# SebastianBitsch/SRGAN-ST

Measured on AMD Instinct MI355X. Metric: HR images/sec (96px x4, B=16/GPU) G+D+ST-loss step, higher is better.
Workload: dtype f32; 1 GPU; srgan_x4_hr96_b16_G+D+ST-loss step: adv+mse+st, D updated every step (train.py:116-164; BASELINE metric); global_batch=16, hr=96, lr=24, parallelism=dp1, hip_graph=True, d_update_interval=1, d_sr_forward=run: all three discriminator forwards of train.py:136,155,158

## Files before the change

srgan-st_amd/csrc/linear.hip:

```cpp
#include "common.h"

typedef float f32x4 __attribute__((ext_vector_type(4)));

namespace {
constexpr int NT = 256;
constexpr int MAXM = 64;

__global__ __launch_bounds__(NT) void linear_fwd_kernel(const float* __restrict__ x, const float* __restrict__ w,
                                                        float* __restrict__ slab, int M, int N, int K, int kslice) {
  __shared__ float red[4][MAXM][17];
  const int wave = __builtin_amdgcn_readfirstlane(threadIdx.x >> 6), lane = threadIdx.x & 63;
  const int lj = lane & 15, lq = lane >> 4;
  const int n0 = blockIdx.x * 16;
  const int kb = blockIdx.y * kslice, ke = min(K, kb + kslice);
  const int mt = (M + 15) / 16;
  f32x4 acc[4];
#pragma unroll
  for (int t = 0; t < 4; ++t) acc[t] = f32x4{0.f, 0.f, 0.f, 0.f};
  const int n = min(n0 + lj, N - 1);
  const float* wrow = w + (size_t)n * K;
  for (int k = kb + wave * 16; k < ke; k += 64) {
    const int kk = k + 4 * lq;
    f32x4 bv = {0.f, 0.f, 0.f, 0.f};
    if (kk + 3 < ke) {
      bv = *reinterpret_cast<const f32x4*>(wrow + kk);
    } else {
#pragma unroll
      for (int j = 0; j < 4; ++j)
        if (kk + j < ke) bv[j] = wrow[kk + j];
    }
#pragma unroll
    for (int t = 0; t < 4; ++t) {
      if (t < mt) {
        const int m = t * 16 + lj;
        f32x4 av = {0.f, 0.f, 0.f, 0.f};
        if (m < M) {
          if (kk + 3 < ke) {
            av = *reinterpret_cast<const f32x4*>(x + (size_t)m * K + kk);
          } else {
#pragma unroll
            for (int j = 0; j < 4; ++j)
              if (kk + j < ke) av[j] = x[(size_t)m * K + kk + j];
          }
        }
#pragma unroll
        for (int j = 0; j < 4; ++j) acc[t] = __builtin_amdgcn_mfma_f32_16x16x4f32(av[j], bv[j], acc[t], 0, 0, 0);
      }
    }
  }
#pragma unroll
  for (int t = 0; t < 4; ++t)
#pragma unroll
    for (int r = 0; r < 4; ++r) red[wave][t * 16 + 4 * lq + r][lj] = acc[t][r];
  __syncthreads();
  for (int i = threadIdx.x; i < M * 16; i += NT) {
    const int m = i >> 4, j = i & 15;
    if (n0 + j < N)
      slab[((size_t)blockIdx.y * M + m) * N + n0 + j] = red[0][m][j] + red[1][m][j] + red[2][m][j] + red[3][m][j];
  }
}

__global__ __launch_bounds__(NT) void linear_reduce_kernel(const float* __restrict__ slab, const float* __restrict__ bias,
                                                           float* __restrict__ y, int nslab, int M, int N) {
  const int total = M * N;
  for (int i = blockIdx.x * NT + threadIdx.x; i < total; i += gridDim.x * NT) {
    float t = bias ? bias[i % N] : 0.f;
    for (int s = 0; s < nslab; ++s) t += slab[(size_t)s * total + i];
    y[i] = t;
  }
}

template <int MT>
__global__ __launch_bounds__(NT) void linear_dgrad_kernel(const float* __restrict__ dy, const float* __restrict__ w,
                                                          float* __restrict__ dx, int M, int N, int K, int C, int HW) {
  __shared__ float red[4][16][65];
  const int wave = __builtin_amdgcn_readfirstlane(threadIdx.x >> 6), lane = threadIdx.x & 63;
  const int lj = lane & 15, lq = lane >> 4;
  const int k0 = blockIdx.x * 64;
  const int nper = ((N + 3) / 4 + 3) / 4 * 4;
  const int nb = wave * nper, ne = min(N, nb + nper);
  f32x4 acc[MT][4];
#pragma unroll
  for (int mt = 0; mt < MT; ++mt)
#pragma unroll
    for (int t = 0; t < 4; ++t) acc[mt][t] = f32x4{0.f, 0.f, 0.f, 0.f};
  int n = nb;
  if (k0 + 64 <= K) {
    constexpr int U = MT == 1 ? 8 : 4;
    const float* wcol = w + k0 + 4 * lj;
    for (; n + 4 * U <= ne; n += 4 * U) {
      f32x4 bv[U];
      float av[MT][U];
#pragma unroll
      for (int u = 0; u < U; ++u) {
        const int nn = n + 4 * u + lq;
        bv[u] = *reinterpret_cast<const f32x4*>(wcol + (size_t)nn * K);
#pragma unroll
        for (int mt = 0; mt < MT; ++mt) {
          const int m = mt * 16 + lj;
          av[mt][u] = m < M ? dy[(size_t)m * N + nn] : 0.f;
        }
      }
#pragma unroll
      for (int u = 0; u < U; ++u)
#pragma unroll
        for (int mt = 0; mt < MT; ++mt)
#pragma unroll
          for (int t = 0; t < 4; ++t) acc[mt][t] = __builtin_amdgcn_mfma_f32_16x16x4f32(av[mt][u], bv[u][t], acc[mt][t], 0, 0, 0);
    }
  }
  for (; n < ne; n += 4) {
    const int nn = n + lq;
    f32x4 bv = {0.f, 0.f, 0.f, 0.f};
    if (nn < ne) {
      const int kk = k0 + 4 * lj;
      if (kk + 3 < K) {
        bv = *reinterpret_cast<const f32x4*>(w + (size_t)nn * K + kk);
      } else {
#pragma unroll
        for (int j = 0; j < 4; ++j)
          if (kk + j < K) bv[j] = w[(size_t)nn * K + kk + j];
      }
    }
#pragma unroll
    for (int mt = 0; mt < MT; ++mt) {
      const int m = mt * 16 + lj;
      const float av = (nn < ne && m < M) ? dy[(size_t)m * N + nn] : 0.f;
#pragma unroll
      for (int t = 0; t < 4; ++t) acc[mt][t] = __builtin_amdgcn_mfma_f32_16x16x4f32(av, bv[t], acc[mt][t], 0, 0, 0);
    }
  }
#pragma unroll
  for (int mt = 0; mt < MT; ++mt) {
    __syncthreads();
#pragma unroll
    for (int t = 0; t < 4; ++t)
#pragma unroll
      for (int r = 0; r < 4; ++r) red[wave][4 * lq + r][4 * lj + t] = acc[mt][t][r];
    __syncthreads();
    for (int i = threadIdx.x; i < 16 * 64; i += NT) {
      const int mm = i >> 6, kc = i & 63, mg = mt * 16 + mm, k = k0 + kc;
      if (mg < M && k < K) {
        const float v = red[0][mm][kc] + red[1][mm][kc] + red[2][mm][kc] + red[3][mm][kc];
        const size_t o = HW > 0 ? (size_t)mg * K + (size_t)(k % HW) * C + k / HW : (size_t)mg * K + k;
        dx[o] = v;
      }
    }
  }
}

__global__ __launch_bounds__(NT) void linear_wgrad_kernel(const float* __restrict__ dy, const float* __restrict__ x,
                                                          float* __restrict__ dw, int M, int N, int K, int accumulate) {
  __shared__ float sdy[MAXM][16];
  const int n0 = blockIdx.y * 16;
  for (int i = threadIdx.x; i < M * 16; i += NT) {
    const int m = i >> 4, j = i & 15;
    sdy[m][j] = (n0 + j < N) ? dy[(size_t)m * N + n0 + j] : 0.f;
  }
  __syncthreads();
  const int k = (blockIdx.x * NT + threadIdx.x) * 4;
  if (k >= K) return;
  const bool vec = (K & 3) == 0;
  f32x4 acc[16];
#pragma unroll
  for (int j = 0; j < 16; ++j) acc[j] = f32x4{0.f, 0.f, 0.f, 0.f};
  for (int m = 0; m < M; ++m) {
    f32x4 xv = {0.f, 0.f, 0.f, 0.f};
    if (vec) {
      xv = *reinterpret_cast<const f32x4*>(x + (size_t)m * K + k);
    } else {
#pragma unroll
      for (int j = 0; j < 4; ++j)
        if (k + j < K) xv[j] = x[(size_t)m * K + k + j];
    }
#pragma unroll
    for (int j = 0; j < 16; ++j) acc[j] += sdy[m][j] * xv;
  }
#pragma unroll
  for (int j = 0; j < 16; ++j) {
    if (n0 + j >= N) break;
    float* d = dw + (size_t)(n0 + j) * K + k;
    if (vec) {
      f32x4 o = acc[j];
      if (accumulate) o += *reinterpret_cast<f32x4*>(d);
      *reinterpret_cast<f32x4*>(d) = o;
    } else {
      for (int q = 0; q < 4; ++q)
        if (k + q < K) d[q] = accumulate ? d[q] + acc[j][q] : acc[j][q];
    }
  }
}

typedef float f32x16 __attribute__((ext_vector_type(16)));
__global__ __launch_bounds__(NT) void linear_wgrad_mfma_kernel(const float* __restrict__ dy, const float* __restrict__ x,
                                                               float* __restrict__ dw, int M, int N, int K, int accumulate) {
  const int wave = threadIdx.x >> 6, lane = threadIdx.x & 63;
  const int li = lane & 31, lh = lane >> 5;
  const int k0 = (blockIdx.x * 4 + wave) * 32, n0 = blockIdx.y * 64;
  if (k0 >= K) return;
  f32x16 acc0, acc1;
#pragma unroll
  for (int r = 0; r < 16; ++r) acc0[r] = acc1[r] = 0.f;
  const float* xp = x + (size_t)lh * K + k0 + li;
  const float* dp = dy + (size_t)lh * N + n0 + li;
  const int steps = (M + 1) >> 1;
  for (int j0 = 0; j0 < steps; j0 += 8) {
    float xv[8], d0[8], d1[8];
#pragma unroll
    for (int u = 0; u < 8; ++u) {
      const int m = 2 * (j0 + u) + lh;
      const bool ok = j0 + u < steps && m < M;
      xv[u] = ok ? xp[(size_t)2 * (j0 + u) * K] : 0.f;
      d0[u] = ok ? dp[(size_t)2 * (j0 + u) * N] : 0.f;
      d1[u] = ok ? dp[(size_t)2 * (j0 + u) * N + 32] : 0.f;
    }
#pragma unroll
    for (int u = 0; u < 8; ++u) {
      acc0 = __builtin_amdgcn_mfma_f32_32x32x2f32(d0[u], xv[u], acc0, 0, 0, 0);
      acc1 = __builtin_amdgcn_mfma_f32_32x32x2f32(d1[u], xv[u], acc1, 0, 0, 0);
    }
  }
#pragma unroll
  for (int r = 0; r < 16; ++r) {
    const int row = (r & 3) + 8 * (r >> 2) + 4 * lh;
    float* d = dw + (size_t)(n0 + row) * K + k0 + li;
    float* e = d + (size_t)32 * K;
    if (accumulate) {
      *d += acc0[r];
      *e += acc1[r];
    } else {
      *d = acc0[r];
      *e = acc1[r];
    }
  }
}

__global__ void colsum_small_kernel(const float* __restrict__ dy, float* __restrict__ db, int M, int N, int accumulate) {
  const int n = blockIdx.x * blockDim.x + threadIdx.x;
  if (n < N) {
    float t = 0.f;
    for (int m = 0; m < M; ++m) t += dy[(size_t)m * N + n];
    db[n] = accumulate ? db[n] + t : t;
  }
}

__global__ __launch_bounds__(NT) void head_fwd_kernel(const float* __restrict__ h, const float* __restrict__ w,
                                                      const float* __restrict__ b, float* __restrict__ y, int M, int N, int K,
                                                      float slope) {
  __shared__ float red[NT / 64];
  const int m = blockIdx.x / N, n = blockIdx.x - m * N;
  float s = 0.f;
  for (int k = threadIdx.x; k < K; k += NT) {
    float v = h[(size_t)m * K + k];
    v = v > 0.f ? v : v * slope;
    s = fmaf(v, w[(size_t)n * K + k], s);
  }
  s = block_sum<NT>(s, red);
  if (threadIdx.x == 0) y[(size_t)m * N + n] = s + (b ? b[n] : 0.f);
}

constexpr int HB_ROWS = 8;
__global__ __launch_bounds__(NT) void head_bwd_kernel(const float* __restrict__ h, const float* __restrict__ w,
                                                      const float* __restrict__ dy, float* __restrict__ dh,
                                                      float* __restrict__ dw, float* __restrict__ db, int M, int N, int K,
                                                      float slope, int accumulate) {
  const int k = blockIdx.x * NT + threadIdx.x;
  const int m0 = blockIdx.y * HB_ROWS, m1 = min(M, m0 + HB_ROWS);
  if (k < K) {
    float hv[HB_ROWS];
#pragma unroll
    for (int i = 0; i < HB_ROWS; ++i) hv[i] = m0 + i < m1 ? h[(size_t)(m0 + i) * K + k] : 0.f;
    float t[HB_ROWS];
#pragma unroll
    for (int i = 0; i < HB_ROWS; ++i) t[i] = 0.f;
    for (int n = 0; n < N; ++n) {
      const float wv = w[(size_t)n * K + k];
#pragma unroll
      for (int i = 0; i < HB_ROWS; ++i)
        if (m0 + i < m1) t[i] = fmaf(dy[(size_t)(m0 + i) * N + n], wv, t[i]);
    }
#pragma unroll
    for (int i = 0; i < HB_ROWS; ++i)
      if (m0 + i < m1) dh[(size_t)(m0 + i) * K + k] = hv[i] > 0.f ? t[i] : t[i] * slope;
    if (dw && blockIdx.y == 0) {
      for (int n = 0; n < N; ++n) {
        float a = 0.f;
        for (int mb = 0; mb < M; mb += HB_ROWS) {
          float v[HB_ROWS];
#pragma unroll
          for (int i = 0; i < HB_ROWS; ++i) v[i] = mb + i < M ? h[(size_t)(mb + i) * K + k] : 0.f;
#pragma unroll
          for (int i = 0; i < HB_ROWS; ++i) {
            if (mb + i >= M) break;
            const float x = v[i] > 0.f ? v[i] : v[i] * slope;
            a = fmaf(dy[(size_t)(mb + i) * N + n], x, a);
          }
        }
        dw[(size_t)n * K + k] = accumulate ? dw[(size_t)n * K + k] + a : a;
      }
    }
  }
  if (db && blockIdx.x == 0 && blockIdx.y == 0 && threadIdx.x < N) {
    float t = 0.f;
    for (int m = 0; m < M; ++m) t += dy[(size_t)m * N + threadIdx.x];
    db[threadIdx.x] = accumulate ? db[threadIdx.x] + t : t;
  }
}

__global__ __launch_bounds__(NT) void flatten_act_kernel(const float* __restrict__ y, const float* __restrict__ scale,
                                                         const float* __restrict__ shift, float slope, int act,
                                                         float* __restrict__ flat, int B, int HW, int C, int gB) {
  const int64_t total = (int64_t)B * HW * C;
  for (int64_t i = blockIdx.x * (int64_t)NT + threadIdx.x; i < total; i += (int64_t)gridDim.x * NT) {
    const int c = (int)(i % C);
    const int64_t p = i / C;
    const int hw = (int)(p % HW);
    const int64_t b = p / HW;
    float v = y[i];
    if (scale) {
      const int gc = (int)(b / gB) * C + c;
      v = fmaf(v, scale[gc], shift[gc]);
    }
    if (act) v = v > 0.f ? v : v * slope;
    flat[(b * C + c) * HW + hw] = v;
  }
}
}

SST_API int sst_linear_ksplit(int M, int N, int K) {
  int ks = 1024 / ((N + 15) / 16);
  if (ks < 1) ks = 1;
  while (ks > 1 && K / ks < 256) ks >>= 1;
  return ks;
}

SST_API int sst_linear_fwd(const float* x, const float* w, const float* bias, float* y, float* slab, int M, int N, int K,
                           void* stream) {
  SST_REQUIRE(x && w && y && slab && M > 0 && M <= MAXM && N > 0 && K > 0, "sst_linear_fwd: bad argument (M=%d)", M);
  const int ks = sst_linear_ksplit(M, N, K);
  const int kslice = ((K + ks - 1) / ks + 63) / 64 * 64;
  dim3 grid((N + 15) / 16, (K + kslice - 1) / kslice);
  linear_fwd_kernel<<<grid, NT, 0, sst_stream(stream)>>>(x, w, slab, M, N, K, kslice);
  SST_LAUNCH_CHECK("linear_fwd_kernel");
  const int rb = (M * N + NT - 1) / NT;
  linear_reduce_kernel<<<rb < 512 ? rb : 512, NT, 0, sst_stream(stream)>>>(slab, bias, y, grid.y, M, N);
  SST_LAUNCH_CHECK("linear_reduce_kernel");
  return SST_OK;
}

SST_API int sst_linear_dgrad(const float* dy, const float* w, float* dx, int M, int N, int K, int nhwc_C, int nhwc_HW,
                             void* stream) {
  SST_REQUIRE(dy && w && dx && M > 0 && M <= MAXM && N > 0 && K > 0, "sst_linear_dgrad: bad argument");
  SST_REQUIRE(nhwc_HW == 0 || nhwc_C * nhwc_HW == K, "sst_linear_dgrad: C*HW must equal K");
  const int grid = (K + 63) / 64;
  hipStream_t st = sst_stream(stream);
  switch ((M + 15) / 16) {
    case 1: linear_dgrad_kernel<1><<<grid, NT, 0, st>>>(dy, w, dx, M, N, K, nhwc_C, nhwc_HW); break;
    case 2: linear_dgrad_kernel<2><<<grid, NT, 0, st>>>(dy, w, dx, M, N, K, nhwc_C, nhwc_HW); break;
    case 3: linear_dgrad_kernel<3><<<grid, NT, 0, st>>>(dy, w, dx, M, N, K, nhwc_C, nhwc_HW); break;
    default: linear_dgrad_kernel<4><<<grid, NT, 0, st>>>(dy, w, dx, M, N, K, nhwc_C, nhwc_HW); break;
  }
  SST_LAUNCH_CHECK("linear_dgrad_kernel");
  return SST_OK;
}

SST_API int sst_linear_wgrad(const float* dy, const float* x, float* dw, float* db, int M, int N, int K, int accumulate,
                             void* stream) {
  SST_REQUIRE(dy && x && dw && M > 0 && M <= MAXM && N > 0 && K > 0, "sst_linear_wgrad: bad argument");
  if ((K & 31) == 0 && (N & 63) == 0 && !sst_env("SST_LINEAR_WGRAD_FMA")) {
    linear_wgrad_mfma_kernel<<<dim3((K / 32 + 3) / 4, N / 64), NT, 0, sst_stream(stream)>>>(dy, x, dw, M, N, K, accumulate);
    SST_LAUNCH_CHECK("linear_wgrad_mfma_kernel");
  } else {
    dim3 grid((K + 4 * NT - 1) / (4 * NT), (N + 15) / 16);
    linear_wgrad_kernel<<<grid, NT, 0, sst_stream(stream)>>>(dy, x, dw, M, N, K, accumulate);
    SST_LAUNCH_CHECK("linear_wgrad_kernel");
  }
  if (db) {
    colsum_small_kernel<<<(N + 255) / 256, 256, 0, sst_stream(stream)>>>(dy, db, M, N, accumulate);
    SST_LAUNCH_CHECK("colsum_small_kernel");
  }
  return SST_OK;
}

SST_API int sst_head_fwd(const float* h, const float* w, const float* b, float* y, int M, int N, int K, float slope,
                         void* stream) {
  SST_REQUIRE(h && w && y && M > 0 && N > 0 && N <= 64 && K > 0, "sst_head_fwd: bad argument");
  head_fwd_kernel<<<M * N, NT, 0, sst_stream(stream)>>>(h, w, b, y, M, N, K, slope);
  SST_LAUNCH_CHECK("head_fwd_kernel");
  return SST_OK;
}

SST_API int sst_head_bwd(const float* h, const float* w, const float* dy, float* dh, float* dw, float* db, int M, int N,
                         int K, float slope, int accumulate, void* stream) {
  SST_REQUIRE(h && w && dy && dh && M > 0 && N > 0 && N <= 64 && K > 0, "sst_head_bwd: bad argument");
  head_bwd_kernel<<<dim3((K + NT - 1) / NT, (M + HB_ROWS - 1) / HB_ROWS), NT, 0, sst_stream(stream)>>>(h, w, dy, dh, dw, db, M, N, K, slope,
                                                                                                    accumulate);
  SST_LAUNCH_CHECK("head_bwd_kernel");
  return SST_OK;
}

SST_API int sst_flatten_act_grp(const float* y, const float* scale, const float* shift, float slope, int act, float* flat,
                                int B, int HW, int C, int grp_images, void* stream) {
  SST_REQUIRE(y && flat && B > 0 && HW > 0 && C > 0 && ((scale == nullptr) == (shift == nullptr)), "sst_flatten_act: bad argument");
  SST_REQUIRE(grp_images >= 0 && (grp_images == 0 || B % grp_images == 0), "sst_flatten_act: bad group size %d for B=%d", grp_images, B);
  const int64_t total = (int64_t)B * HW * C;
  const int blocks = (int)((total + NT - 1) / NT < 2048 ? (total + NT - 1) / NT : 2048);
  flatten_act_kernel<<<blocks, NT, 0, sst_stream(stream)>>>(y, scale, shift, slope, act, flat, B, HW, C, grp_images > 0 ? grp_images : B);
  SST_LAUNCH_CHECK("flatten_act_kernel");
  return SST_OK;
}
```

Baseline: 3262 HR images/s.

## Batch loads ahead of MFMA in linear kernels and fuse bias-grad colsum

Result: no change. 3279 HR images/s (median of 6 runs) (+0.5%).

```diff
diff --git a/srgan-st_amd/csrc/linear.hip b/srgan-st_amd/csrc/linear.hip
--- a/srgan-st_amd/csrc/linear.hip
+++ b/srgan-st_amd/csrc/linear.hip
@@ -6,50 +6,70 @@
 constexpr int NT = 256;
 constexpr int MAXM = 64;
 
+#define LOADS_FIRST() __builtin_amdgcn_sched_barrier(0)
+
+constexpr int FWD_STEP = 16;
+constexpr int fwd_unroll(int MT) { return MT <= 2 ? 6 : 3; }
+template <int MT>
 __global__ __launch_bounds__(NT) void linear_fwd_kernel(const float* __restrict__ x, const float* __restrict__ w,
                                                         float* __restrict__ slab, int M, int N, int K, int kslice) {
-  __shared__ float red[4][MAXM][17];
+  __shared__ float red[4][16 * MT][17];
+  constexpr int U = fwd_unroll(MT);
   const int wave = __builtin_amdgcn_readfirstlane(threadIdx.x >> 6), lane = threadIdx.x & 63;
   const int lj = lane & 15, lq = lane >> 4;
   const int n0 = blockIdx.x * 16;
   const int kb = blockIdx.y * kslice, ke = min(K, kb + kslice);
-  const int mt = (M + 15) / 16;
-  f32x4 acc[4];
-#pragma unroll
-  for (int t = 0; t < 4; ++t) acc[t] = f32x4{0.f, 0.f, 0.f, 0.f};
-  const int n = min(n0 + lj, N - 1);
-  const float* wrow = w + (size_t)n * K;
-  for (int k = kb + wave * 16; k < ke; k += 64) {
+  const int seg = kslice >> 2;
+  const int wb = kb + wave * seg, we = min(ke, wb + seg);
+  f32x4 acc[MT];
+#pragma unroll
+  for (int t = 0; t < MT; ++t) acc[t] = f32x4{0.f, 0.f, 0.f, 0.f};
+  const float* wrow = w + (size_t)min(n0 + lj, N - 1) * K + 4 * lq;
+  const float* xrow[MT];
+#pragma unroll
+  for (int t = 0; t < MT; ++t) xrow[t] = x + (size_t)min(t * 16 + lj, M - 1) * K + 4 * lq;
+  int k = wb;
+  for (; k + FWD_STEP * U <= we; k += FWD_STEP * U) {
+    f32x4 bv[U], av[MT][U];
+#pragma unroll
+    for (int u = 0; u < U; ++u) {
+      bv[u] = *reinterpret_cast<const f32x4*>(wrow + k + FWD_STEP * u);
+#pragma unroll
+      for (int t = 0; t < MT; ++t) av[t][u] = *reinterpret_cast<const f32x4*>(xrow[t] + k + FWD_STEP * u);
+    }
+    LOADS_FIRST();
+#pragma unroll
+    for (int u = 0; u < U; ++u)
+#pragma unroll
+      for (int t = 0; t < MT; ++t)
+#pragma unroll
+        for (int j = 0; j < 4; ++j) acc[t] = __builtin_amdgcn_mfma_f32_16x16x4f32(av[t][u][j], bv[u][j], acc[t], 0, 0, 0);
+  }
+  for (; k < we; k += FWD_STEP) {
     const int kk = k + 4 * lq;
-    f32x4 bv = {0.f, 0.f, 0.f, 0.f};
-    if (kk + 3 < ke) {
-      bv = *reinterpret_cast<const f32x4*>(wrow + kk);
+    f32x4 bv = {0.f, 0.f, 0.f, 0.f}, av[MT];
+#pragma unroll
+    for (int t = 0; t < MT; ++t) av[t] = f32x4{0.f, 0.f, 0.f, 0.f};
+    if (kk + 3 < we) {
+      bv = *reinterpret_cast<const f32x4*>(wrow + k);
+#pragma unroll
+      for (int t = 0; t < MT; ++t) av[t] = *reinterpret_cast<const f32x4*>(xrow[t] + k);
     } else {
 #pragma unroll
       for (int j = 0; j < 4; ++j)
-        if (kk + j < ke) bv[j] = wrow[kk + j];
-    }
-#pragma unroll
-    for (int t = 0; t < 4; ++t) {
-      if (t < mt) {
-        const int m = t * 16 + lj;
-        f32x4 av = {0.f, 0.f, 0.f, 0.f};
-        if (m < M) {
-          if (kk + 3 < ke) {
-            av = *reinterpret_cast<const f32x4*>(x + (size_t)m * K + kk);
-          } else {
-#pragma unroll
-            for (int j = 0; j < 4; ++j)
-              if (kk + j < ke) av[j] = x[(size_t)m * K + kk + j];
-          }
+        if (kk + j < we) {
+          bv[j] = wrow[k + j];
+#pragma unroll
+          for (int t = 0; t < MT; ++t) av[t][j] = xrow[t][k + j];
         }
-#pragma unroll
-        for (int j = 0; j < 4; ++j) acc[t] = __builtin_amdgcn_mfma_f32_16x16x4f32(av[j], bv[j], acc[t], 0, 0, 0);
-      }
-    }
-  }
-#pragma unroll
-  for (int t = 0; t < 4; ++t)
+    }
+#pragma unroll
+    for (int t = 0; t < MT; ++t)
+#pragma unroll
+      for (int j = 0; j < 4; ++j) acc[t] = __builtin_amdgcn_mfma_f32_16x16x4f32(av[t][j], bv[j], acc[t], 0, 0, 0);
+  }
+#pragma unroll
+  for (int t = 0; t < MT; ++t)
 #pragma unroll
     for (int r = 0; r < 4; ++r) red[wave][t * 16 + 4 * lq + r][lj] = acc[t][r];
   __syncthreads();
@@ -60,23 +80,36 @@
   }
 }
 
+constexpr int RED_U = 8;
 __global__ __launch_bounds__(NT) void linear_reduce_kernel(const float* __restrict__ slab, const float* __restrict__ bias,
                                                            float* __restrict__ y, int nslab, int M, int N) {
   const int total = M * N;
   for (int i = blockIdx.x * NT + threadIdx.x; i < total; i += gridDim.x * NT) {
     float t = bias ? bias[i % N] : 0.f;
-    for (int s = 0; s < nslab; ++s) t += slab[(size_t)s * total + i];
+    int s = 0;
+    for (; s + RED_U <= nslab; s += RED_U) {
+      float v[RED_U];
+#pragma unroll
+      for (int u = 0; u < RED_U; ++u) v[u] = slab[(size_t)(s + u) * total + i];
+      LOADS_FIRST();
+#pragma unroll
+      for (int u = 0; u < RED_U; ++u) t += v[u];
+    }
+    for (; s < nslab; ++s) t += slab[(size_t)s * total + i];
     y[i] = t;
   }
 }
 
+constexpr int DG_CB = 64;
+constexpr int DG_ROWS = 4;
+constexpr int DG_U = 8;
 template <int MT>
 __global__ __launch_bounds__(NT) void linear_dgrad_kernel(const float* __restrict__ dy, const float* __restrict__ w,
                                                           float* __restrict__ dx, int M, int N, int K, int C, int HW) {
-  __shared__ float red[4][16][65];
+  __shared__ float red[4][16][DG_CB + 1];
   const int wave = __builtin_amdgcn_readfirstlane(threadIdx.x >> 6), lane = threadIdx.x & 63;
   const int lj = lane & 15, lq = lane >> 4;
-  const int k0 = blockIdx.x * 64;
+  const int k0 = blockIdx.x * DG_CB;
   const int nper = ((N + 3) / 4 + 3) / 4 * 4;
   const int nb = wave * nper, ne = min(N, nb + nper);
   f32x4 acc[MT][4];
@@ -85,31 +118,30 @@
 #pragma unroll
     for (int t = 0; t < 4; ++t) acc[mt][t] = f32x4{0.f, 0.f, 0.f, 0.f};
   int n = nb;
-  if (k0 + 64 <= K) {
-    constexpr int U = MT == 1 ? 8 : 4;
-    const float* wcol = w + k0 + 4 * lj;
-    for (; n + 4 * U <= ne; n += 4 * U) {
-      f32x4 bv[U];
-      float av[MT][U];
-#pragma unroll
-      for (int u = 0; u < U; ++u) {
-        const int nn = n + 4 * u + lq;
-        bv[u] = *reinterpret_cast<const f32x4*>(wcol + (size_t)nn * K);
-#pragma unroll
-        for (int mt = 0; mt < MT; ++mt) {
-          const int m = mt * 16 + lj;
-          av[mt][u] = m < M ? dy[(size_t)m * N + nn] : 0.f;
-        }
-      }
-#pragma unroll
-      for (int u = 0; u < U; ++u)
+  if (k0 + DG_CB <= K) {
+    const float* wcol = w + (size_t)(DG_U * lq) * K + k0 + 4 * lj;
+    const float* drow[MT];
+#pragma unroll
+    for (int mt = 0; mt < MT; ++mt) drow[mt] = dy + (size_t)min(mt * 16 + lj, M - 1) * N + DG_U * lq;
+    for (; n + DG_ROWS * DG_U <= ne; n += DG_ROWS * DG_U) {
+      f32x4 bv[DG_U], aq[MT][DG_U / 4];
+#pragma unroll
+      for (int mt = 0; mt < MT; ++mt)
+#pragma unroll
+        for (int q = 0; q < DG_U / 4; ++q) aq[mt][q] = *reinterpret_cast<const f32x4*>(drow[mt] + n + 4 * q);
+#pragma unroll
+      for (int u = 0; u < DG_U; ++u) bv[u] = *reinterpret_cast<const f32x4*>(wcol + (size_t)(n + u) * K);
+      if constexpr (MT == 1) LOADS_FIRST();
+#pragma unroll
+      for (int u = 0; u < DG_U; ++u)
 #pragma unroll
         for (int mt = 0; mt < MT; ++mt)
 #pragma unroll
-          for (int t = 0; t < 4; ++t) acc[mt][t] = __builtin_amdgcn_mfma_f32_16x16x4f32(av[mt][u], bv[u][t], acc[mt][t], 0, 0, 0);
-    }
-  }
-  for (; n < ne; n += 4) {
+          for (int t = 0; t < 4; ++t)
+            acc[mt][t] = __builtin_amdgcn_mfma_f32_16x16x4f32(aq[mt][u >> 2][u & 3], bv[u][t], acc[mt][t], 0, 0, 0);
+    }
+  }
+  for (; n < ne; n += DG_ROWS) {
     const int nn = n + lq;
     f32x4 bv = {0.f, 0.f, 0.f, 0.f};
     if (nn < ne) {
@@ -138,8 +170,8 @@
 #pragma unroll
       for (int r = 0; r < 4; ++r) red[wave][4 * lq + r][4 * lj + t] = acc[mt][t][r];
     __syncthreads();
-    for (int i = threadIdx.x; i < 16 * 64; i += NT) {
-      const int mm = i >> 6, kc = i & 63, mg = mt * 16 + mm, k = k0 + kc;
+    for (int i = threadIdx.x; i < 16 * DG_CB; i += NT) {
+      const int mm = i / DG_CB, kc = i % DG_CB, mg = mt * 16 + mm, k = k0 + kc;
       if (mg < M && k < K) {
         const float v = red[0][mm][kc] + red[1][mm][kc] + red[2][mm][kc] + red[3][mm][kc];
         const size_t o = HW > 0 ? (size_t)mg * K + (size_t)(k % HW) * C + k / HW : (size_t)mg * K + k;
@@ -150,7 +182,8 @@
 }
 
 __global__ __launch_bounds__(NT) void linear_wgrad_kernel(const float* __restrict__ dy, const float* __restrict__ x,
-                                                          float* __restrict__ dw, int M, int N, int K, int accumulate) {
+                                                          float* __restrict__ dw, float* __restrict__ db, int M, int N, int K,
+                                                          int accumulate) {
   __shared__ float sdy[MAXM][16];
   const int n0 = blockIdx.y * 16;
   for (int i = threadIdx.x; i < M * 16; i += NT) {
@@ -158,6 +191,11 @@
     sdy[m][j] = (n0 + j < N) ? dy[(size_t)m * N + n0 + j] : 0.f;
   }
   __syncthreads();
+  if (db && blockIdx.x == 0 && threadIdx.x < 16 && n0 + threadIdx.x < N) {
+    float t = 0.f;
+    for (int m = 0; m < M; ++m) t += sdy[m][threadIdx.x];
+    db[n0 + threadIdx.x] = accumulate ? db[n0 + threadIdx.x] + t : t;
+  }
   const int k = (blockIdx.x * NT + threadIdx.x) * 4;
   if (k >= K) return;
   const bool vec = (K & 3) == 0;
@@ -191,56 +229,67 @@
   }
 }
 
+constexpr int WG_KW = 32;
+constexpr int WG_NB = 64;
+constexpr int WG_PAIRS = 8;
 typedef float f32x16 __attribute__((ext_vector_type(16)));
 __global__ __launch_bounds__(NT) void linear_wgrad_mfma_kernel(const float* __restrict__ dy, const float* __restrict__ x,
-                                                               float* __restrict__ dw, int M, int N, int K, int accumulate) {
-  const int wave = threadIdx.x >> 6, lane = threadIdx.x & 63;
-  const int li = lane & 31, lh = lane >> 5;
-  const int k0 = (blockIdx.x * 4 + wave) * 32, n0 = blockIdx.y * 64;
-  if (k0 >= K) return;
-  f32x16 acc0, acc1;
-#pragma unroll
-  for (int r = 0; r < 16; ++r) acc0[r] = acc1[r] = 0.f;
-  const float* xp = x + (size_t)lh * K + k0 + li;
-  const float* dp = dy + (size_t)lh * N + n0 + li;
-  const int steps = (M + 1) >> 1;
-  for (int j0 = 0; j0 < steps; j0 += 8) {
-    float xv[8], d0[8], d1[8];
-#pragma unroll
-    for (int u = 0; u < 8; ++u) {
-      const int m = 2 * (j0 + u) + lh;
-      const bool ok = j0 + u < steps && m < M;
-      xv[u] = ok ? xp[(size_t)2 * (j0 + u) * K] : 0.f;
-      d0[u] = ok ? dp[(size_t)2 * (j0 + u) * N] : 0.f;
-      d1[u] = ok ? dp[(size_t)2 * (j0 + u) * N + 32] : 0.f;
-    }
-#pragma unroll
-    for (int u = 0; u < 8; ++u) {
-      acc0 = __builtin_amdgcn_mfma_f32_32x32x2f32(d0[u], xv[u], acc0, 0, 0, 0);
-      acc1 = __builtin_amdgcn_mfma_f32_32x32x2f32(d1[u], xv[u], acc1, 0, 0, 0);
-    }
-  }
-#pragma unroll
-  for (int r = 0; r < 16; ++r) {
-    const int row = (r & 3) + 8 * (r >> 2) + 4 * lh;
-    float* d = dw + (size_t)(n0 + row) * K + k0 + li;
-    float* e = d + (size_t)32 * K;
+                                                               float* __restrict__ dw, float* __restrict__ db, int M, int N, int K,
+                                                               int accumulate) {
+  const int wave = __builtin_amdgcn_readfirstlane(threadIdx.x >> 6), lane = threadIdx.x & 63;
+  const int lh = lane >> 5;
+  const unsigned li = lane & 31;
+  const int k0 = (blockIdx.x * 4 + wave) * WG_KW, n0 = blockIdx.y * WG_NB;
+  if (k0 < K) {
+    f32x16 acc0, acc1;
+#pragma unroll
+    for (int r = 0; r < 16; ++r) acc0[r] = acc1[r] = 0.f;
+    const int steps = (M + 1) >> 1;
+    for (int j0 = 0; j0 < steps; j0 += WG_PAIRS) {
+      float xv[WG_PAIRS], d0[WG_PAIRS], d1[WG_PAIRS];
+#pragma unroll
+      for (int u = 0; u < WG_PAIRS; ++u) {
+        const int j2 = min(2 * (j0 + u), M - 1), one = 2 * (j0 + u) + lh < M ? lh : 0;
+        xv[u] = (x + (size_t)j2 * K + k0)[one * K + li];
+        const float* dp = dy + (size_t)j2 * N + n0;
+        d0[u] = dp[one * N + li];
+        d1[u] = dp[one * N + li + 32];
+      }
+      LOADS_FIRST();
+#pragma unroll
+      for (int u = 0; u < WG_PAIRS; ++u) {
+        const bool ok = 2 * (j0 + u) + lh < M;
+        const float xu = ok ? xv[u] : 0.f;
+        acc0 = __builtin_amdgcn_mfma_f32_32x32x2f32(ok ? d0[u] : 0.f, xu, acc0, 0, 0, 0);
+        acc1 = __builtin_amdgcn_mfma_f32_32x32x2f32(ok ? d1[u] : 0.f, xu, acc1, 0, 0, 0);
+      }
+    }
+    float* const d = dw + (size_t)n0 * K + k0 + (4 * lh * K + li);
+    const auto row = [K](int r) { return (size_t)((r & 3) + 8 * (r >> 2)) * K; };
     if (accumulate) {
-      *d += acc0[r];
-      *e += acc1[r];
+      float o[16];
+#pragma unroll
+      for (int r = 0; r < 16; ++r) o[r] = d[row(r)];
+      LOADS_FIRST();
+#pragma unroll
+      for (int r = 0; r < 16; ++r) d[row(r)] = o[r] + acc0[r];
+#pragma unroll
+      for (int r = 0; r < 16; ++r) o[r] = d[row(r) + (size_t)32 * K];
+      LOADS_FIRST();
+#pragma unroll
+      for (int r = 0; r < 16; ++r) d[row(r) + (size_t)32 * K] = o[r] + acc1[r];
     } else {
-      *d = acc0[r];
-      *e = acc1[r];
-    }
-  }
-}
-
-__global__ void colsum_small_kernel(const float* __restrict__ dy, float* __restrict__ db, int M, int N, int accumulate) {
-  const int n = blockIdx.x * blockDim.x + threadIdx.x;
-  if (n < N) {
+#pragma unroll
+      for (int r = 0; r < 16; ++r) {
+        d[row(r)] = acc0[r];
+        d[row(r) + (size_t)32 * K] = acc1[r];
+      }
+    }
+  }
+  if (db && blockIdx.x == 0 && wave == 0) {
     float t = 0.f;
-    for (int m = 0; m < M; ++m) t += dy[(size_t)m * N + n];
-    db[n] = accumulate ? db[n] + t : t;
+    for (int m = 0; m < M; ++m) t += dy[(size_t)m * N + n0 + lane];
+    db[n0 + lane] = accumulate ? db[n0 + lane] + t : t;
   }
 }
 
@@ -340,10 +389,16 @@
   const int ks = sst_linear_ksplit(M, N, K);
   const int kslice = ((K + ks - 1) / ks + 63) / 64 * 64;
   dim3 grid((N + 15) / 16, (K + kslice - 1) / kslice);
-  linear_fwd_kernel<<<grid, NT, 0, sst_stream(stream)>>>(x, w, slab, M, N, K, kslice);
+  hipStream_t st = sst_stream(stream);
+  switch ((M + 15) / 16) {
+    case 1: linear_fwd_kernel<1><<<grid, NT, 0, st>>>(x, w, slab, M, N, K, kslice); break;
+    case 2: linear_fwd_kernel<2><<<grid, NT, 0, st>>>(x, w, slab, M, N, K, kslice); break;
+    case 3: linear_fwd_kernel<3><<<grid, NT, 0, st>>>(x, w, slab, M, N, K, kslice); break;
+    default: linear_fwd_kernel<4><<<grid, NT, 0, st>>>(x, w, slab, M, N, K, kslice); break;
+  }
   SST_LAUNCH_CHECK("linear_fwd_kernel");
   const int rb = (M * N + NT - 1) / NT;
-  linear_reduce_kernel<<<rb < 512 ? rb : 512, NT, 0, sst_stream(stream)>>>(slab, bias, y, grid.y, M, N);
+  linear_reduce_kernel<<<rb < 512 ? rb : 512, NT, 0, st>>>(slab, bias, y, grid.y, M, N);
   SST_LAUNCH_CHECK("linear_reduce_kernel");
   return SST_OK;
 }
@@ -352,8 +407,8 @@
                              void* stream) {
   SST_REQUIRE(dy && w && dx && M > 0 && M <= MAXM && N > 0 && K > 0, "sst_linear_dgrad: bad argument");
   SST_REQUIRE(nhwc_HW == 0 || nhwc_C * nhwc_HW == K, "sst_linear_dgrad: C*HW must equal K");
-  const int grid = (K + 63) / 64;
   hipStream_t st = sst_stream(stream);
+  const int grid = (K + DG_CB - 1) / DG_CB;
   switch ((M + 15) / 16) {
     case 1: linear_dgrad_kernel<1><<<grid, NT, 0, st>>>(dy, w, dx, M, N, K, nhwc_C, nhwc_HW); break;
     case 2: linear_dgrad_kernel<2><<<grid, NT, 0, st>>>(dy, w, dx, M, N, K, nhwc_C, nhwc_HW); break;
@@ -368,16 +423,12 @@
                              void* stream) {
   SST_REQUIRE(dy && x && dw && M > 0 && M <= MAXM && N > 0 && K > 0, "sst_linear_wgrad: bad argument");
   if ((K & 31) == 0 && (N & 63) == 0 && !sst_env("SST_LINEAR_WGRAD_FMA")) {
-    linear_wgrad_mfma_kernel<<<dim3((K / 32 + 3) / 4, N / 64), NT, 0, sst_stream(stream)>>>(dy, x, dw, M, N, K, accumulate);
+    linear_wgrad_mfma_kernel<<<dim3((K / WG_KW + 3) / 4, N / WG_NB), NT, 0, sst_stream(stream)>>>(dy, x, dw, db, M, N, K, accumulate);
     SST_LAUNCH_CHECK("linear_wgrad_mfma_kernel");
   } else {
     dim3 grid((K + 4 * NT - 1) / (4 * NT), (N + 15) / 16);
-    linear_wgrad_kernel<<<grid, NT, 0, sst_stream(stream)>>>(dy, x, dw, M, N, K, accumulate);
+    linear_wgrad_kernel<<<grid, NT, 0, sst_stream(stream)>>>(dy, x, dw, db, M, N, K, accumulate);
     SST_LAUNCH_CHECK("linear_wgrad_kernel");
-  }
-  if (db) {
-    colsum_small_kernel<<<(N + 255) / 256, 256, 0, sst_stream(stream)>>>(dy, db, M, N, accumulate);
-    SST_LAUNCH_CHECK("colsum_small_kernel");
   }
   return SST_OK;
 }
```
